# zertovitch/zip-ada

Measured on AMD Instinct MI355X. Metric: Deflate encode MB/s (Deflate_3; stream bit-exact with the CPU restatement of the reference, Ada parity unpinned), higher is better.
Workload: dtype u8

## Files before the change

### zip-ada_amd/csrc/zada_api.hip

```cpp
#include <hip/hip_runtime.h>
#include <stdint.h>
#include <stdio.h>
#include <string.h>
#include <algorithm>
#include <new>
#include <atomic>
#include <mutex>
#include <condition_variable>
#include <functional>
#include <thread>
#include "../../include/zada.h"
#include "zada_internal.h"
#include "zada_bt4.h"

struct zada_ctx { zada::Ctx c; };

namespace zada {

thread_local std::string *tls_err = nullptr;
int hip_check(Ctx *c, hipError_t e, const char *what) {
  if (e == hipSuccess) return 0;
  char buf[256];
  snprintf(buf, sizeof buf, "%s: %s", what, hipGetErrorString(e));
  if (tls_err) *tls_err = buf; else c->err = buf;
// ... 889 lines not shown
  unlzma_destroy(&z->c);
  lzma_free(&z->c);
  free_workspace(&z->c);
  for (hipEvent_t e : z->c.ev_pool) hipEventDestroy(e);
  if (z->c.stream2) hipStreamDestroy(z->c.stream2);
  if (z->c.crc_host) hipHostFree(z->c.crc_host);
  for (int b = 0; b < 2 * MAX_COPY_LANES; b++) { if (z->c.stage[b]) hipHostFree(z->c.stage[b]); if (z->c.ev_stage[b]) hipEventDestroy(z->c.ev_stage[b]); }
  for (int t = 0; t < MAX_COPY_LANES; t++) { if (z->c.stream_in[t]) hipStreamDestroy(z->c.stream_in[t]); if (z->c.ev_in[t]) hipEventDestroy(z->c.ev_in[t]); }
  if (z->c.bstage) hipHostFree(z->c.bstage);
  if (z->c.btab) hipHostFree(z->c.btab);
  if (z->c.ev_input) hipEventDestroy(z->c.ev_input);
  if (z->c.ev_out) hipEventDestroy(z->c.ev_out);
  if (z->c.ev_dlim) hipEventDestroy(z->c.ev_dlim);
  if (z->c.stream) hipStreamDestroy(z->c.stream);
  delete z;
}

zada_ctx *zada_create(int device) {
  int ndev = 0;
  if (hipGetDeviceCount(&ndev) != hipSuccess || ndev <= 0 || device < 0 || device >= ndev) return nullptr;
  if (hipSetDevice(device) != hipSuccess) return nullptr;
  zada_ctx *z = new (std::nothrow) zada_ctx();
  if (!z) return nullptr;
  z->c.device = device;
  if (hipStreamCreate(&z->c.stream) != hipSuccess ||
      hipHostMalloc((void **)&z->c.crc_host, (CRC_HOST_TOP + 64) * 4, hipHostMallocDefault) != hipSuccess ||
      hipStreamCreate(&z->c.stream2) != hipSuccess || hipEventCreateWithFlags(&z->c.ev_input, hipEventDisableTiming) != hipSuccess ||
      hipEventCreateWithFlags(&z->c.ev_out, hipEventDisableTiming) != hipSuccess || hipEventCreateWithFlags(&z->c.ev_dlim, hipEventDisableTiming) != hipSuccess) { (void)hipGetLastError(); ctx_release(z); return nullptr; }
  if (const char *e = getenv("ZADA_BUDGET")) z->c.knob_budget = atoi(e);
  if (const char *e = getenv("ZADA_INNER_BUDGET")) z->c.knob_inner_budget = atoi(e);
  if (const char *e = getenv("ZADA_LINK_RUN")) { const int v = atoi(e); if (v >= 0 && v <= 64 && !(v & (v - 1))) z->c.knob_link_run = v; }
  if (const char *e = getenv("ZADA_ATOMS_PCT")) { if (atoi(e) >= 1 && atoi(e) <= 100) z->c.knob_atoms_pct = atoi(e); }
  if (const char *e = getenv("ZADA_CD_FILTER")) z->c.knob_cd_filter = atoi(e) != 0;
  if (const char *e = getenv("ZADA_EXACT_RESPEC")) { if (atoi(e) >= 0) z->c.knob_exact_respec = atoi(e); }
  if (const char *e = getenv("ZADA_MAX_DEMAND_ROUNDS")) { if (atoi(e) > 0) z->c.knob_max_demand_rounds = atoi(e); }
  if (const char *e = getenv("ZADA_SHARD_KIB")) { if (atoi(e) >= 64 && atoi(e) % 64 == 0) z->c.knob_shard_kib = atoi(e); }
  return z;
}

void zada_destroy(zada_ctx *z) {
  if (!z) return;
  hipSetDevice(z->c.device);
  ctx_release(z);
}

const char *zada_last_error(const zada_ctx *z) { return z ? z->c.err.c_str() : "no context"; }

int zada_set_knob(zada_ctx *z, const char *name, int value) {
  if (!z || !name) return ZADA_E_INVALID;
  if (!strcmp(name, "budget")) z->c.knob_budget = value;
  else if (!strcmp(name, "inner_budget")) z->c.knob_inner_budget = value;
  else if (!strcmp(name, "link_run")) { if (value < 0 || value > 64 || (value & (value - 1))) return ZADA_E_INVALID; z->c.knob_link_run = value; }
  else if (!strcmp(name, "span_mib")) { if (value < 1 || value > 3968) return ZADA_E_INVALID; z->c.knob_span_mib = value; }
  else if (!strcmp(name, "bunzip_batch_mib")) { if (value < 16 || value > 262144) return ZADA_E_INVALID; z->c.knob_bunzip_batch_mib = value; }
  else if (!strcmp(name, "bz_batch_mib")) { if (value < 1 || value > 2048) return ZADA_E_INVALID; z->c.knob_bz_batch_mib = value; }
  else if (!strcmp(name, "bz_span_mib")) { if (value < 24 || value > 3072) return ZADA_E_INVALID; z->c.knob_bz_span_mib = value; }
  else if (!strcmp(name, "bz_batch_melems")) { if (value < 1 || value > 1536) return ZADA_E_INVALID; z->c.knob_bz_batch_melems = value; }
  else if (!strcmp(name, "bz_tail_pct")) { if (value < 0 || value > 50) return ZADA_E_INVALID; z->c.knob_bz_tail_pct = value; }
  else if (!strcmp(name, "bz_text_order")) { if (value < 0 || value > 1) return ZADA_E_INVALID; z->c.knob_bz_text_order = value; }
  else if (!strcmp(name, "bz_pipeline")) { if (value < 0 || value > 1) return ZADA_E_INVALID; z->c.knob_bz_pipeline = value; }
  else if (!strcmp(name, "bz_pipe_prio")) { if (value < 0 || value > 1) return ZADA_E_INVALID; z->c.knob_bz_pipe_prio = value; }
  else if (!strcmp(name, "bz_list_rows")) { if (value < 0 || value > 8192) return ZADA_E_INVALID; z->c.knob_bz_list_rows = value; }
  else if (!strcmp(name, "bz_split")) { if (value < 0 || value > 1) return ZADA_E_INVALID; z->c.knob_bz_split = value; }
  else if (!strcmp(name, "bz_small_wg")) { if (value < 0 || value > 1) return ZADA_E_INVALID; z->c.knob_bz_small_wg = value; }
  else if (!strcmp(name, "bz_lists")) { if (value < -1) return ZADA_E_INVALID; z->c.knob_bz_lists = value; }
  else if (!strcmp(name, "batch_mib")) { if (value < 1 || value > 1024) return ZADA_E_INVALID; z->c.knob_batch_mib = value; }
  else if (!strcmp(name, "atoms_pct")) { if (value < 1 || value > 100) return ZADA_E_INVALID; z->c.knob_atoms_pct = value; z->c.ws.cap_atoms = 0; }
  else if (!strcmp(name, "fix_stride")) { if (value < 0 || value > (int)PTOK_STRIDE) return ZADA_E_INVALID; z->c.knob_fix_stride = value; z->c.ws.cap_n = 0; }
  else if (!strcmp(name, "cd_list_cap")) { if (value < 0) return ZADA_E_INVALID; z->c.knob_cd_list_cap = value; }
  else if (!strcmp(name, "cd_filter")) { if (value < 0 || value > 1) return ZADA_E_INVALID; z->c.knob_cd_filter = value; }
  else if (!strcmp(name, "exact_respec")) { if (value < 0) return ZADA_E_INVALID; z->c.knob_exact_respec = value; }
  else if (!strcmp(name, "max_demand_rounds")) z->c.knob_max_demand_rounds = value > 0 ? value : 12;
  else if (!strcmp(name, "shard_kib")) { if (value < 64 || value % 64) return ZADA_E_INVALID; z->c.knob_shard_kib = value; }
  else if (!strcmp(name, "lzma_dict")) { if (value < 0) return ZADA_E_INVALID; z->c.knob_lzma_dict = value; }
  else if (!strcmp(name, "lzma_chunk")) { if (value < -1 || (value > 0 && value < 256)) return ZADA_E_INVALID; z->c.knob_lzma_chunk = value; }
  else if (!strcmp(name, "lzma_pool")) { if (value < 0) return ZADA_E_INVALID; z->c.knob_lzma_pool = value; }
  else if (!strcmp(name, "lzma_pool_fixed")) { if (value < 0 || value > 1) return ZADA_E_INVALID; z->c.knob_lzma_pool_fixed = value; }
  else if (!strcmp(name, "lzma_waves")) { if (value != 0 && value != 1 && value != 4) return ZADA_E_INVALID; z->c.knob_lzma_waves = value; }
  else if (!strcmp(name, "lzma_lit_mib")) { if (value < 1) return ZADA_E_INVALID; z->c.knob_lzma_lit_mib = value; }
  else if (!strcmp(name, "lzma_segment")) { if (value < -1 || (value > 0 && (value < 13 || value > 30))) return ZADA_E_INVALID; z->c.knob_lzma_segment = value; }
  else return ZADA_E_INVALID;
  return ZADA_OK;
}

constexpr int COPY_LANES = ZADA_COPY_LANES;
static_assert(COPY_LANES <= MAX_COPY_LANES, "staging buffers");
static_assert(COPY_LANES == ARR_LANES, "the arriving input's lanes use the staging buffers of copy_in's");
constexpr uint64_t COPY_MT_MIN = 64ull << 20;
static bool ensure_staging(Ctx *c, int lanes) {
  for (int b = 0; b < 2 * lanes; b++) {
    if (c->stage[b]) continue;
    if (hipHostMalloc((void **)&c->stage[b], STAGE_BYTES, hipHostMallocDefault) != hipSuccess ||
        hipEventCreateWithFlags(&c->ev_stage[b], hipEventDisableTiming) != hipSuccess) {
      if (c->stage[b]) { hipHostFree(c->stage[b]); c->stage[b] = nullptr; }
      (void)hipGetLastError();
      return false;
    }
  }
  return true;
}

static void copy_in_lane(Ctx *c, void *d_dst, const uint8_t *src, uint64_t n, int t, int T) {
  uint64_t i = 0;
// ... 1165 lines not shown
```

### zip-ada_amd/csrc/zada_internal.h

```cpp
#pragma once
#ifndef ZADA_NLEVELS
#define ZADA_NLEVELS 2
#endif
#include <hip/hip_runtime.h>
#include <stdint.h>
#include <string>
#include <functional>
#include <vector>
#include "zada_logic.h"
#include "zada_sizing.h"

namespace zada {

constexpr int ZADA_E_HIP_ = -3;

#ifndef ZADA_PCHUNK
#define ZADA_PCHUNK 512
#endif
constexpr uint32_t PCHUNK = ZADA_PCHUNK;
static_assert(PCHUNK > 258, "k_fix_forward: a 258-byte step crosses at most one chunk boundary");
constexpr uint32_t PTOK_STRIDE = PCHUNK + 640;
constexpr uint32_t FIX_STRIDE_SMALL = 128;
constexpr uint32_t CRC_CHUNK = 4096, CRC_SUB = 256;
constexpr uint64_t IN_PAD = 1024;
// ... 203 lines not shown
  void *bzd = nullptr;
  void *ulz = nullptr;
  void *lz_tab = nullptr; size_t cap_lz_tab = 0;
  void *lz_save = nullptr; size_t cap_lz_save = 0;
  void *lz_lit = nullptr; size_t cap_lz_lit = 0;
  bool lz_last_lit_hbm = false;
  int knob_lzma_lit_mib = 12288;
  int lzma_launches = 0;
  std::vector<uint8_t> lz_resume;
  bool lz_stopped = false;
  bool lz_run_stopped = false;
  uint64_t lz_last_n = 0, lz_last_out_off = 0;
  void *bt4 = nullptr;
  uint32_t bt4_buckets = 0, bt4_long = 0, bt4_overflow = 0;
  uint32_t bt4_pool_grown = 0;
  int knob_lzma_pool_fixed = 0;
  uint32_t bt4_reruns = 0;
  int knob_lzma_waves = 0;
  int knob_lzma_segment = 0;
  int knob_lzma_pool = 0;
  std::vector<hipEvent_t> ev_pool;
  std::vector<std::pair<const char *, hipEvent_t>> marks;
  std::vector<std::pair<const char *, float>> timing;
  bool timing_on = true;
  uint32_t last_nblocks = 0;
  int knob_budget = -1;
  int knob_max_demand_rounds = 12;
  int knob_atoms_pct = 50;
  int knob_fix_stride = 0;
  int knob_cd_list_cap = 0;
  int knob_cd_filter = 1;
  int knob_exact_respec = 32768;
  int knob_bz_pipe_prio = 0;
  int knob_link_run = 0;
  int knob_inner_budget = 0;
  int knob_span_mib = 2048;
  int knob_batch_mib = 512;
  int knob_bunzip_batch_mib = 8192;
  int knob_bz_batch_mib = 256;
  int knob_bz_span_mib = 1024;
  int knob_bz_text_order = 1;
  int knob_bz_tail_pct = 0;
  int knob_bz_batch_melems = 768;
  int knob_bz_lists = -1;
  int knob_bz_pipeline = 1;
  int knob_bz_list_rows = 0;
  int knob_bz_split = 1;
  int knob_bz_small_wg = 1;
  int knob_lzma_dict = 0;
  int knob_lzma_chunk = 0;
  int knob_shard_kib = 1 << 20;
  void tmark(const char *name);
  void tbegin();
  void tend();
};

extern thread_local std::string *tls_err;
int hip_check(Ctx *c, hipError_t e, const char *what);
void bz2_destroy(Ctx *c);
void crypt_destroy(Ctx *c);
void inflate_destroy(Ctx *c);
int inflate_crc_entries(Ctx *c, uint32_t E, const uint64_t *out, const uint64_t *out_len, uint32_t *regs);
void bunzip2_destroy(Ctx *c);
void unlzma_destroy(Ctx *c);
void crypt_update_keys(uint32_t keys[3], uint8_t by);
uint8_t crypt_code(const uint32_t keys[3]);
// ... 76 lines not shown
```

### zip-ada_amd/csrc/zada_lz.hip

```cpp
#include <hip/hip_runtime.h>
#include <mutex>
#include <stdint.h>
#include "zada_logic.h"
#include "zada_internal.h"
#include <chrono>
#include <stdio.h>
#include <stdlib.h>
#include <vector>

namespace zada {

typedef uint32_t __attribute__((aligned(1))) u32u;
typedef uint64_t __attribute__((aligned(1))) u64u;
#define RL(v, j) ((uint32_t)__builtin_amdgcn_readlane((int)(v), (j)))
#define RL64(v, j) ((uint64_t)RL((uint32_t)(v), (j)) | ((uint64_t)RL((uint32_t)((v) >> 32), (j)) << 32))

#ifndef ZADA_NO_XCD_MAP
__device__ __forceinline__ uint32_t xcd_block() {
  const uint32_t n = gridDim.x, full = n & ~7u, b = blockIdx.x;
  return b < full ? (b & 7u) * (full >> 3) + (b >> 3) : b;
}
#else
__device__ __forceinline__ uint32_t xcd_block() { return blockIdx.x; }
#endif
// ... 92 lines not shown
    for (int k = 0; k < w; k++) base += wsum[k];
    uint32_t run = base + incl - s;
    for (int k = 0; k < PER; k++) { const int idx = tid * PER + k; cnt[(idx & 15) * NDIG + (idx >> 4)] = run; run += v[k]; }
  }
  lds_barrier();
  SP_STAMP(2);
#pragma unroll
  for (int it = 0; it < 32; it++) {
    if (it * 64 < rem) {
      const uint32_t wd = word(it), d = (wd >> (16 + SHIFT)) & (uint32_t)(NDIG - 1);
      dst[mycnt[d] + ((rk[it >> 1] >> (16 * (it & 1))) & 0xFFFFu)] = wd;
    }
  }
  lds_barrier();
  SP_STAMP(3);
}

constexpr uint32_t DIST3_CONTINUE = 0xFFFF, DIST3_HEADCHK = 0xFFFE, DIST3_CONT_FIRST = 0xFFFD, DISTL_CONTINUE = 0x8000;
#ifndef ZADA_WALK_CAP
#define ZADA_WALK_CAP 16
#endif
constexpr uint32_t DISTL_GAVEUP = 0x7FFF, WALK_CAP = ZADA_WALK_CAP;
static_assert(MAX_DIST < 0x7FFF, "the give-up marker is no distance");
constexpr uint32_t HEAVY_STRIDE = 2048, HEAVY_CAP = HEAVY_STRIDE - 1;
static_assert(MAX_DIST < 0x8000, "continue markers of the planes");
constexpr int PL_LDS = 144 * 1024 + 64, PL_LDS_RUNS = 160 * 1024, PL_PREV_OFF = 131072;
constexpr int PL_HB_OFF = PL_PREV_OFF + 12288;
static_assert(PL_PREV_OFF + 32768 <= PL_LDS_RUNS, "k_prev_links: LDS map of the fused cross links");
template <bool RUNS>
__global__ void __launch_bounds__(1024) k_prev_links(const uint8_t *__restrict__ in, Layout L, int kfull, int kquarter,
                                                     LevelPtrs lv,
                                                     uint16_t *__restrict__ S3, uint8_t *__restrict__ T3, uint32_t *__restrict__ bsc3,
                                                     DistPlanes dp, RunPtrs rp, unsigned long long *__restrict__ dbg, uint32_t *__restrict__ segmax,
                                                     uint16_t *__restrict__ heavy, uint32_t seg0, uint32_t run_len, uint32_t seg_end) {
#ifdef ZADA_PL_STATS
  unsigned long long tprev = clock64(); int tph = 8;
#define PL_STAMP() do { lds_barrier(); if (threadIdx.x == 0) { unsigned long long t = clock64(); atomicAdd(&dbg[tph], t - tprev); tprev = t; } tph++; } while (0)
#else
#define PL_STAMP() do {} while (0)
#endif
  extern __shared__ __attribute__((aligned(16))) uint8_t smem[];
  uint16_t *A = (uint16_t *)smem;
  uint16_t *B = A + 32768;
  uint32_t *AB = (uint32_t *)smem;
  uint32_t *cnt = (uint32_t *)(B + 32768);
  uint32_t *wsum = cnt + 4096;
  const int tid = threadIdx.x, lane = tid & 63, w = tid >> 6;
  const uint8_t *pbL = smem + PL_PREV_OFF;
#pragma unroll 1
  for (uint32_t jrun = 0; jrun < (RUNS ? run_len : 1u); jrun++) {
  const uint64_t seg = (uint64_t)blockIdx.x * run_len + jrun + seg0, base = seg * 32768ull;
  if (seg >= seg_end) break;
  const uint32_t m = lay_inserted(L, seg);
  const bool first_seg = lay_first(L, seg);
  const bool fused = RUNS && jrun > 0 && !first_seg;
  const bool prev_first = fused && lay_first(L, seg - 1);

#ifdef ZADA_PL_STATS
  tph = 8;
#endif
  uint32_t *bsc = bsc3 + seg * 32768ull;
  uint16_t *s3 = S3 + seg * 32768ull;
  uint8_t *t3 = T3 + seg * 32768ull;
  uint16_t *hvy = heavy + seg * HEAVY_STRIDE;
  const uint32_t heavy_thr = kquarter / 2 > 0 ? (uint32_t)kquarter / 2 : 1u;
#ifdef ZADA_OLD_INIT
  for (int l = 0; l < NLEVELS; l++) {
    uint16_t *tail = lv.tails[l] + seg * 65536ull;
    for (int i = tid; i < 65536 / 8; i += 1024) ((uint4 *)tail)[i] = make_uint4(~0u, ~0u, ~0u, ~0u);
  }
  for (uint32_t e = tid; e < m; e += 1024) dp.dlim[base + e] = 0xFFFFFFFFu;
#endif
  const uint8_t *sin = in + base;
  PL_STAMP();
  uint32_t *F = cnt;
  uint16_t *LW = (uint16_t *)(cnt + 1040);
  const uint8_t *sb = (const uint8_t *)A;
  uint16_t *P = B;
  auto lb8 = [&](uint32_t e) -> uint64_t {
    const uint32_t *wp = (const uint32_t *)(sb + (e & ~3u));
    const uint32_t a = wp[0], b = wp[1], s = e & 3u;
    return (uint64_t)__builtin_amdgcn_alignbyte(b, a, s) | ((uint64_t)(b >> (8u * s)) << 32);
  };
  static_assert(3 + NLEVELS <= 5 + 1, "lb8 yields five valid bytes");
#pragma unroll 1
  for (int lvl = 0; lvl <= NLEVELS; lvl++) {
    const int L = 3 + lvl;
    uint32_t i0 = (uint32_t)w * 2048 + lane;
    asm volatile("" : "+v"(i0));
    const int rem = (int)m - (int)i0;

    {
      {
        uint32_t key[16];
#pragma unroll
        for (int k = 0; k < 16; k++) key[k] = 0;
        const uint32_t sh = i0 & 3u;
        auto build = [&](auto wp) {
#pragma unroll
          for (int g8 = 0; g8 < 4; g8++) {
            uint32_t wa[8], wb[8], wc[8];
#pragma unroll
            for (int q = 0; q < 8; q++) { const int it = g8 * 8 + q; wa[q] = wp[it * 16]; wb[q] = wp[it * 16 + 1]; wc[q] = wp[it * 16 + 2]; }
#pragma unroll
            for (int q = 0; q < 8; q++) {
              const int it = g8 * 8 + q;
              const uint64_t v = (uint64_t)__builtin_amdgcn_alignbyte(wb[q], wa[q], sh) | ((uint64_t)__builtin_amdgcn_alignbyte(wc[q], wb[q], sh) << 32);
              uint32_t k = (lvl == 0) ? hash3_of(v) : hashL_of(v, L);
              if (!(it * 64 < rem)) k = 0;
              key[it >> 1] |= k << (16 * (it & 1));
            }
          }
        };
        if (lvl == 0) {
          build((const uint32_t *)(sin + (i0 & ~3u)));
          for (int i = tid; i < 32768 / 4; i += 1024) ((uint4 *)bsc)[i] = make_uint4(0, 0, 0, 0);
          if (RUNS) {
            for (int l = 0; l < NLEVELS; l++) {
              uint16_t *tl = lv.tails[l] + seg * 65536ull;
              for (int i = tid; i < 65536 / 8; i += 1024) ((uint4 *)tl)[i] = make_uint4(~0u, ~0u, ~0u, ~0u);
            }
          }
        } else build((const uint32_t *)(sb + (i0 & ~3u)));
        sort_pass<256, 0, true>(key, AB, cnt, wsum, i0, rem);
      }
      uint32_t pr[32];
      {
        const uint32_t *pp = AB + i0;
#pragma unroll
        for (int it = 0; it < 32; it++) pr[it] = (it * 64 < rem) ? pp[it * 64] : 0u;
      }
      if (lvl == 0) sort_pass<128, 8, false>(pr, AB, cnt, wsum, i0, rem);
      else sort_pass<256, 8, false>(pr, AB, cnt, wsum, i0, rem);
    }
    if (lvl == 0) __syncthreads();
    PL_STAMP();
    uint16_t *tail = lvl > 0 ? lv.tails[lvl - 1] + seg * 65536ull : nullptr;
    const bool want_runs = lvl == 0 || lvl == NLEVELS;
    uint32_t ed[32];
    const bool keyed = RUNS && fused && lvl > 0;
    uint32_t *HB = (uint32_t *)(smem + PL_HB_OFF);
    uint32_t firstmask = 0;
    if (keyed) HB[tid] = 0;
    {
      const uint32_t *pp = AB + i0;
      uint32_t *pf = F + (i0 >> 5);
#pragma unroll
      for (int it = 0; it < 32; it++) {
        uint32_t x = 0;
        bool first = false;
        if (it * 64 < rem) {
          const uint32_t p0 = pp[it * 64], e = p0 & 0xFFFFu, k = p0 >> 16;
          uint32_t pm = 0;
          first = i0 + it * 64 == 0;
          if (!first) { pm = pp[it * 64 - 1]; first = (pm >> 16) != k; }
          const bool last = (it * 64 + 1 == rem) || ((pp[it * 64 + 1] >> 16) != k);
          uint32_t d = 0;
          if (!first) { const uint32_t e0 = pm & 0xFFFFu; if (!(first_seg && e0 == 0)) d = e - e0; }
          else if (keyed) d = k;
          firstmask |= (uint32_t)first << it;
          x = e | ((uint32_t)last << 15) | (d << 16);
          if (lvl > 0 && last) tail[k] = (uint16_t)e;
        }
        ed[it] = x;
        if (want_runs) {
          const unsigned long long mk = __ballot(first);
          if (lane == 0) { pf[it * 2] = (uint32_t)mk; pf[it * 2 + 1] = (uint32_t)(mk >> 32); }
        }
// ... 107 lines not shown
              P[eb[q]] = (t != 0xFFFFu && dx <= (uint32_t)MAX_DIST && !(prev_first && t == 0)) ? (uint16_t)dx : (uint16_t)0;
            }
          }
        }
        lds_barrier();
        if (lvl < NLEVELS) { for (uint32_t i = tid; i < (m + 16 + 15) / 16; i += 1024) ((uint4 *)A)[i] = ((const uint4 *)sin)[i]; }
      }
      uint16_t *prevl = lv.prev[lvl - 1];
      for (uint32_t i = tid; i < (m + 7) / 8; i += 1024) ((uint4 *)(prevl + base))[i] = ((const uint4 *)P)[i];
    }
    PL_STAMP();
    if (lvl < NLEVELS) {
      const uint64_t lmask = (1ull << (8 * L)) - 1ull;
      uint16_t *plane = dp.d[lvl] + base;
      auto dflt_of = [&](uint32_t e, uint32_t q) -> uint32_t {
        if (first_seg) return 0u;
        if (lvl == 0) return e < (uint32_t)TOO_FAR ? (q == e ? DIST3_CONT_FIRST : DIST3_CONTINUE) : (q == e ? DIST3_HEADCHK : 0u);
        if (RUNS && fused) {
          const uint32_t step = P[q];
          if (step == 0) return 0u;
          const uint32_t t = q + 32768u - step, d = e + 32768u - t;
          if (d > (uint32_t)MAX_DIST) return 0u;
          if (t <= 32768u - 4u) {
            const uint32_t theirs = lds_u32_tail(pbL, t);
            if (theirs == (uint32_t)lb8(e)) return d;
          }
        }
        return DISTL_CONTINUE | (e - q);
      };
      static_assert(NLEVELS <= 2, "the candidate compare of the fused cross links takes four bytes");
      constexpr uint32_t QCAP = 4000;
      uint32_t *Qa = (uint32_t *)(smem + 32800), *Qb = Qa + QCAP;
      uint32_t *qn = RUNS ? (uint32_t *)(smem + 32800 + 8 * QCAP) : wsum;
      static_assert(32800 + 8 * QCAP + 8 <= 65536, "queues and their counters behind the staged bytes");
      const unsigned long long ltm = (1ull << lane) - 1ull;
      if (tid < 2) qn[tid] = 0;
      if (RUNS && fused && lvl > 0) {
        const uint4 *bs = (const uint4 *)(in + base - 32768ull);
        for (int i = tid; i < 32768 / 16; i += 1024) ((uint4 *)(smem + PL_PREV_OFF))[i] = bs[i];
      }
      lds_barrier();
      auto walk = [&](uint32_t e, uint32_t &q, uint64_t mine, uint32_t maxs, uint32_t &dl) -> bool {
        uint32_t step = P[q];
        for (uint32_t sidx = 0; sidx < maxs; sidx++) {
          if (step - 1u >= q) { dl = dflt_of(e, q); return true; }
          q -= step;
          const uint32_t dist = e - q;
          step = P[q];
          const uint64_t theirs = lb8(q);
          if (dist > (uint32_t)(lvl == 0 ? TOO_FAR : MAX_DIST)) { dl = 0; return true; }
          if ((theirs & lmask) == mine) { dl = dist; return true; }
        }
        return false;
      };
      auto push = [&](bool pend, uint32_t entry, uint32_t *dstq, uint32_t *cntp) -> bool {
        const unsigned long long mk = __ballot(pend);
        if (mk == 0) return true;
        uint32_t b0 = 0;
        const int leader = __ffsll((long long)mk) - 1;
        if (lane == leader) b0 = atomicAdd(cntp, (uint32_t)__popcll(mk));
        b0 = __shfl(b0, leader);
        const uint32_t idx = b0 + __popcll(mk & ltm);
        if (pend && idx < QCAP) { dstq[idx] = entry; return true; }
        return !pend;
      };
      const bool capped = lvl > 0 && !first_seg && WALK_CAP > 0;
      const uint32_t maxs_last = capped ? WALK_CAP : 1u << 30;
      for (uint32_t e0 = 0; e0 < m; e0 += 4096) {
        uint32_t ee[4], st[4];
        uint64_t mn[4], th[4];
        bool ex[4];
#pragma unroll
        for (int j = 0; j < 4; j++) { const uint32_t e = e0 + 1024u * j + tid; ex[j] = e < m; ee[j] = ex[j] ? e : 0u; }
#pragma unroll
        for (int j = 0; j < 4; j++) { mn[j] = lb8(ee[j]) & lmask; st[j] = P[ee[j]]; }
#pragma unroll
        for (int j = 0; j < 4; j++) th[j] = lb8(st[j] <= ee[j] ? ee[j] - st[j] : ee[j]) & lmask;
        uint32_t pw[4] = {0, 0, 0, 0};
        if (RUNS && fused && lvl > 0) {
#pragma unroll
          for (int j = 0; j < 4; j++) {
            const uint32_t t = st[j] > ee[j] ? ee[j] + 32768u - st[j] : 0u, tr = t <= 32768u - 4u ? t : 0u;
            pw[j] = lds_u32_tail(pbL, tr);
          }
        }
#pragma unroll
        for (int j = 0; j < 4; j++) {
          const uint32_t e = ee[j], step = st[j];
          uint32_t dl = 0, q = e;
          bool pend = false;
          if (!(ex[j] && step - 1u < e)) {
            if (RUNS && fused && lvl > 0) {
              if (step != 0) dl = (e + 32768u - step <= 32768u - 4u && pw[j] == (uint32_t)mn[j]) ? step : DISTL_CONTINUE;
            } else dl = dflt_of(e, e);
          }
          if (ex[j] && step - 1u < e) {
            q = e - step;
            if (lvl == 0) {
              if (th[j] == mn[j] && (step <= (uint32_t)TOO_FAR || step == (uint32_t)MAX_DIST)) dl = step;
              else if (step >= (uint32_t)TOO_FAR) dl = 0;
              else pend = true;
            } else {
              if (step > (uint32_t)MAX_DIST) dl = 0;
              else if (th[j] == mn[j]) dl = step;
              else pend = true;
            }
          }
          if (!push(pend, e | (q << 16), Qa, &qn[0])) { if (!walk(e, q, mn[j], maxs_last, dl)) dl = DISTL_GAVEUP; pend = false; }
          if (ex[j] && !pend) plane[e] = (uint16_t)dl;
        }
      }
      lds_barrier();
      PL_STAMP();
      for (int cur = 0;; cur ^= 1) {
        const uint32_t nq = qn[cur] < QCAP ? qn[cur] : QCAP;
        if (nq == 0) break;
#ifdef ZADA_PL_STATS
        if (tid == 0 && lvl == 1) { atomicAdd(&dbg[24], 1ull); atomicAdd(&dbg[25], (unsigned long long)nq); if (nq <= 1024) atomicAdd(&dbg[26], (unsigned long long)nq); if (cur == 0 && qn[0] > QCAP) atomicAdd(&dbg[30], (unsigned long long)(qn[0] - QCAP)); }
        unsigned long long tq0 = clock64();
#endif
        lds_barrier();
        if (tid == 0) qn[cur ^ 1] = 0;
        lds_barrier();
        if (nq > 1024) {
          static_assert(QCAP <= 4096, "four entries per lane cover the queue");
          const uint32_t *Qs = cur ? Qb : Qa;
          uint32_t e4[4], q4[4], st4[4], dl4[4];
          uint64_t mn4[4];
          bool val[4], act[4];
#pragma unroll
          for (int j = 0; j < 4; j++) {
            const uint32_t idx = 1024u * j + tid;
            val[j] = idx < nq;
            const uint32_t ent = Qs[val[j] ? idx : 0u];
            e4[j] = ent & 0x7FFFu; q4[j] = ent >> 16; act[j] = val[j]; dl4[j] = 0;
          }
#pragma unroll
          for (int j = 0; j < 4; j++) { mn4[j] = lb8(e4[j]) & lmask; st4[j] = P[q4[j]]; }
          for (int sidx = 0; sidx < 8; sidx++) {
            uint32_t qx[4], ns[4];
            uint64_t th[4];
#pragma unroll
            for (int j = 0; j < 4; j++) {
// ... 304 lines not shown
    const uint64_t lo = p - (uint64_t)MAX_DIST > first ? p - (uint64_t)MAX_DIST : first;
    const uint32_t mine = *(const u32u *)(in + p);
    uint32_t found = 0;
    for (uint64_t hi = p; hi > lo && !found; hi = hi - lo > 2048 ? hi - 2048 : lo) {
      uint64_t v[8];
#pragma unroll
      for (int u = 0; u < 8; u++) {
        const uint64_t q0 = hi - 256ull * (uint64_t)(u + 1) + 4ull * lane;
        v[u] = (q0 < hi && q0 + 3 >= lo) ? *(const u64u *)(in + q0) : 0ull;
      }
#pragma unroll
      for (int u = 0; u < 8; u++) {
        const uint64_t q0 = hi - 256ull * (uint64_t)(u + 1) + 4ull * lane;
        uint32_t mk = 0;
        if (q0 < hi && q0 + 3 >= lo) {
#pragma unroll
          for (int j = 0; j < 4; j++) if ((uint32_t)(v[u] >> (8 * j)) == mine && q0 + (uint64_t)j >= lo && q0 + (uint64_t)j < hi) mk |= 1u << j;
        }
        const unsigned long long m = __ballot(mk != 0);
        if (m && !found) {
          const int top = 63 - __builtin_clzll(m);
          const uint32_t tm = RL(mk, top);
          const uint64_t q = hi - 256ull * (uint64_t)(u + 1) + 4ull * (uint64_t)top + (uint64_t)(31 - __builtin_clz(tm));
          found = (uint32_t)(p - q);
        }
      }
    }
    if (lane == 0) dp.d[1][p] = (uint16_t)found;
  }
}

__global__ void __launch_bounds__(256) k_bucket_limits(Layout L, int kfull, int kquarter, const uint16_t *__restrict__ S3,
                                                       const uint32_t *__restrict__ bsc3, uint32_t *__restrict__ dlim, uint32_t *__restrict__ dlim_bits, const uint32_t *__restrict__ segmax,
                                                       const uint16_t *__restrict__ heavy, uint32_t seg0) {
  __shared__ uint32_t list[2048];
  __shared__ uint32_t nlist;
  __shared__ uint32_t lbits[1024];
  const uint64_t seg = (uint64_t)blockIdx.x + seg0, base = seg * 32768ull;
  const int tid = threadIdx.x;
  const bool has_prev = !lay_first(L, seg);
  {
    const uint32_t mo = segmax[seg], mp = has_prev ? segmax[seg - 1] : 0u;
    if (mo == 0 || mo - 1 + mp < (uint32_t)kquarter) return;
  }
  for (int i = tid; i < 1024; i += 256) lbits[i] = 0;
  auto flush_bits = [&]() { __syncthreads(); for (int i = tid; i < 1024; i += 256) { const uint32_t w = lbits[i]; if (w) dlim_bits[(base >> 5) + i] = w; } };
  const uint32_t *own = bsc3 + base, *prv = has_prev ? bsc3 + base - 32768 : nullptr;
  const uint16_t *s3 = S3 + base, *p3 = has_prev ? S3 + base - 32768 : nullptr;
  auto qualifies = [&](uint32_t h) -> bool {
    const uint32_t c = own[h] >> 16, cp = prv ? prv[h] >> 16 : 0u;
    return c > 0 && c - 1 + cp >= (uint32_t)kquarter;
  };
  auto process = [&]() {
    const uint32_t nl = nlist < 2048 ? nlist : 2048;
    for (uint32_t li = 0; li < nl; li++) {
      const uint32_t h = list[li];
      const uint32_t st = own[h] & 0xFFFF, c = own[h] >> 16;
      const uint32_t pst = prv ? prv[h] & 0xFFFF : 0u, cp = prv ? prv[h] >> 16 : 0u;
      const uint32_t r0 = (uint32_t)kquarter > cp ? (uint32_t)kquarter - cp : 0u;
      for (uint32_t r = r0 + tid; r < c; r += 256) {
        const uint32_t e = s3[st + r];
        uint32_t lim[2];
        const uint32_t ks[2] = {(uint32_t)kfull, (uint32_t)kquarter};
        for (int t = 0; t < 2; t++) {
          const uint32_t k = ks[t];
          uint64_t d = 0xFFFF;
          if (r >= k) d = e - s3[st + r - k];
          else if (cp >= k - r) d = (base + e) - (base - 32768 + p3[pst + cp - (k - r)]);
          lim[t] = d < 0xFFFF ? (uint32_t)d : 0xFFFFu;
        }
        dlim[base + e] = lim[0] | (lim[1] << 16);
        atomicOr(&lbits[e >> 5], 1u << (e & 31u));
      }
    }
  };
  const uint32_t heavy_thr = kquarter / 2 > 0 ? (uint32_t)kquarter / 2 : 1u;
  const uint16_t *ho = heavy + seg * HEAVY_STRIDE, *hp = has_prev ? heavy + (seg - 1) * HEAVY_STRIDE : nullptr;
  const uint32_t no = ho[0], np = hp ? hp[0] : 0u;
  if (no != 0xFFFFu && np != 0xFFFFu) {
    for (int phase = 0; phase < 2; phase++) {
      if (tid == 0) nlist = 0;
      __syncthreads();
      const uint16_t *hl = phase == 0 ? ho : hp;
      const uint32_t nh = phase == 0 ? no : np;
      for (uint32_t i = tid; i < nh; i += 256) {
        const uint32_t h = hl[1 + i];
        if (phase == 1 && (own[h] >> 16) >= heavy_thr) continue;
        if (qualifies(h)) { const uint32_t k = atomicAdd(&nlist, 1u); if (k < 2048) list[k] = h; }
      }
      __syncthreads();
      process();
      __syncthreads();
    }
    flush_bits();
    return;
  }
  for (uint32_t h0 = 0; h0 < 32768; h0 += 2048) {
    if (tid == 0) nlist = 0;
    __syncthreads();
    for (uint32_t h = h0 + tid; h < h0 + 2048; h += 256) {
      if (qualifies(h)) { const uint32_t k = atomicAdd(&nlist, 1u); if (k < 2048) list[k] = h; }
    }
    __syncthreads();
    process();
    __syncthreads();
// ... 1000 lines not shown
      if (int rg = job.grow_atoms(cnt, &dst_atoms, &dst_apos)) return rg;
    }
    if (cnt) hipLaunchKernelGGL(k_literal_atoms, dim3(2048), dim3(256), 0, st, W.in + job.tok_lo, cnt, dst_atoms, dst_apos, job.apos_bias + job.tok_lo);
    res->ntok = (uint32_t)cnt;
    res->exit = ExitState{(uint32_t)hi, SYNC_F};
    return hip_check(c, hipGetLastError(), "k_literal_atoms");
  }
  const LzConfig cfg = lz_config(level);
  const Layout L{job.segend, n};
  const uint64_t n_ins = job.segend ? n : (n >= 2 ? n - 2 : 0);
  const uint32_t nseg = (uint32_t)((n_ins + 32767) / 32768);
  c->tmark("lz:begin");
  if (!c->lz_attrs_set) {
    hipFuncSetAttribute((const void *)k_prev_links<true>, hipFuncAttributeMaxDynamicSharedMemorySize, PL_LDS_RUNS);
    hipFuncSetAttribute((const void *)k_prev_links<false>, hipFuncAttributeMaxDynamicSharedMemorySize, PL_LDS);
    hipFuncSetAttribute((const void *)k_cross_links, hipFuncAttributeMaxDynamicSharedMemorySize, CL_LDS_PLANE);
    hipFuncSetAttribute((const void *)k_match, hipFuncAttributeMaxDynamicSharedMemorySize, MATCH_LDS);
    hipFuncSetAttribute((const void *)k_match_demand, hipFuncAttributeMaxDynamicSharedMemorySize, DM_LDS);
    c->lz_attrs_set = true;
  }
  LevelPtrs lv;
  DistPlanes dpl;
  RunPtrs rpt; rpt.S = W.SK; rpt.idx = W.idxK; rpt.cnt = W.cntK;
  for (int l = 0; l < NLEVELS; l++) dpl.d[l] = W.dplane[l];
  dpl.dlim = W.dlim; dpl.dlim_bits = W.dlim_bits;
  if (nseg > 0) {
    for (int l = 0; l < NLEVELS; l++) { lv.prev[l] = W.lprev[l]; lv.tails[l] = W.ltails[l]; }
#ifndef ZADA_OLD_INIT
    hipEventRecord(c->ev_dlim, st);
    hipStreamWaitEvent(c->stream2, c->ev_dlim, 0);
    hipMemsetAsync(W.dlim_bits, 0, (size_t)(n / 32 + 2) * 4, c->stream2);
    hipEventRecord(c->ev_dlim, c->stream2);
#endif
    uint32_t R = 1;
    if (c->knob_link_run > 0) R = (uint32_t)c->knob_link_run;
    else {
      while (R < 16 && nseg / (2 * R) >= 1024) R *= 2;
      if (job.need && R > 8) R = 8;
    }
    if ((R & (R - 1)) || R > 64) { c->err = "link_run is not a power of two up to 64"; return -1; }
    auto prev_links = [&](uint32_t s0, uint32_t s1) {
      if (R > 1) hipLaunchKernelGGL(k_prev_links<true>, dim3((s1 - s0 + R - 1) / R), dim3(1024), PL_LDS_RUNS, st, W.in, L, cfg.chain, cfg.chain >> 2, lv,
                                    W.S3, W.T3, W.bsc3, dpl, rpt, (unsigned long long *)W.dbg, W.segmax, W.heavy, s0, R, s1);
      else hipLaunchKernelGGL(k_prev_links<false>, dim3(s1 - s0), dim3(1024), PL_LDS, st, W.in, L, cfg.chain, cfg.chain >> 2, lv,
                              W.S3, W.T3, W.bsc3, dpl, rpt, (unsigned long long *)W.dbg, W.segmax, W.heavy, s0, 1u, s1);
    };
    auto cross_links = [&](uint32_t from, uint32_t to) {
      const uint32_t first = (from + R - 1) / R * R;
      if (first < to) hipLaunchKernelGGL(k_cross_links, dim3((to - first + R - 1) / R, NLEVELS), dim3(1024), CL_LDS_PLANE, st, W.in, L, lv, dpl, first, R);
    };
    static_assert(BLOOM_WORDS == 4096, "Workspace::bloom4 is sized in zada_api.hip");
    auto cross_dist = [&]() {
      const uint32_t nb = (uint32_t)((n_ins - 32768 + CD_THREADS - 1) / CD_THREADS);
      if (!c->knob_cd_filter) {
        hipLaunchKernelGGL(k_cross_dist<CD_ALL>, dim3(nb), dim3(CD_THREADS), 0, st, W.in, L, lv, W.S3, W.T3, W.bsc3, dpl, (uint64_t)32768, (uint64_t)n, CdTail{nullptr, nullptr, W.n_changed + 4, 0u, nullptr, W.n_changed + 5, 0u});
        return;
      }
      hipMemsetAsync(W.n_changed + 4, 0, 4, st);
      hipLaunchKernelGGL(k_bloom4, dim3(nseg - 1), dim3(256), 0, st, W.in, L, W.bloom4, 0u);
      hipMemsetAsync(W.n_changed + 5, 0, 4, st);
      const uint32_t lcap = c->knob_cd_list_cap > 0 && (uint64_t)c->knob_cd_list_cap < W.cd_cap ? (uint32_t)c->knob_cd_list_cap : (uint32_t)W.cd_cap;
      const CdTail tl{W.bloom4, W.cd_list, W.n_changed + 4, lcap, W.cd_list + W.cd_cap, W.n_changed + 5, lcap / 4};
      hipLaunchKernelGGL(k_cross_dist<CD_SWEEP>, dim3(nb), dim3(CD_THREADS), 0, st, W.in, L, lv, W.S3, W.T3, W.bsc3, dpl, (uint64_t)32768, (uint64_t)n, tl);
      hipLaunchKernelGGL(k_cross_dist<CD_LIST>, dim3((uint32_t)((W.cd_cap + CD_THREADS - 1) / CD_THREADS)), dim3(CD_THREADS), 0, st, W.in, L, lv, W.S3, W.T3, W.bsc3, dpl, (uint64_t)0, (uint64_t)n, tl);
      hipLaunchKernelGGL(k_cross_scan, dim3(2048), dim3(256), 0, st, W.in, L, dpl, tl);
    };
    if (job.need) {
      constexpr uint32_t PIECE = 2048;
      static_assert(PIECE % 64 == 0, "pieces start at multiples of every run length (a power of two up to 64)");
      constexpr double SLOW_PIECE_S = 2.0e-3;
      uint32_t cl_from = 1;
      auto cross_links_upto = [&](uint32_t s1) {
        if (s1 > cl_from) cross_links(cl_from, s1);
        if (s1 > cl_from) cl_from = s1;
      };
      auto t_prev = std::chrono::steady_clock::now();
      for (uint32_t s0 = 0; s0 < nseg;) {
        const uint32_t s1 = s0 + PIECE < nseg ? s0 + PIECE : nseg;
        const uint64_t upto = (uint64_t)s1 * 32768 + 64 < n ? (uint64_t)s1 * 32768 + 64 : n;
        if (int rn = job.need(upto)) return rn;
        const auto t_now = std::chrono::steady_clock::now();
        const bool slow = s0 > 0 && std::chrono::duration<double>(t_now - t_prev).count() >= SLOW_PIECE_S;
        t_prev = t_now;
        prev_links(s0, s1);
#ifndef ZADA_OLD_INIT
        if (s0 == 0) hipStreamWaitEvent(st, c->ev_dlim, 0);
#endif
        if (slow) cross_links_upto(s1);
        hipLaunchKernelGGL(k_bucket_limits, dim3(s1 - s0), dim3(256), 0, st, L, cfg.chain, cfg.chain >> 2, W.S3, W.bsc3, W.dlim, W.dlim_bits, W.segmax, W.heavy, s0);
        s0 = s1;
      }
      if (int rn = job.need(n)) return rn;
      cross_links_upto(nseg);
      if (nseg > 1) cross_dist();
    } else
    prev_links(0, nseg);
#ifndef ZADA_OLD_INIT
    if (!job.need) hipStreamWaitEvent(st, c->ev_dlim, 0);
#endif
#ifdef ZADA_PL_STATS
    { unsigned long long h[32]; hipMemcpy(h, W.dbg, sizeof h, hipMemcpyDeviceToHost); fprintf(stderr, "[prev_links cycles/segment] init %.0f |", (double)h[8] / nseg); for (int q = 9; q < 9 + 4 * (NLEVELS + 1) - 1; q++) fprintf(stderr, " %.0f", (double)h[q] / nseg); fprintf(stderr, "  (per level 3..: sort, links, first candidates, queue rounds)\n"); fprintf(stderr, "[level 4 walks per segment] rounds %.2f  entries %.1f  entries of the last round %.1f  hops there %.1f (max %llu over all segments; walks over 64 hops %.3f)  first-queue overflow %.1f  cycles of the last round %.0f\n", (double)h[24] / nseg, (double)h[25] / nseg, (double)h[26] / nseg, (double)h[27] / nseg, h[28], (double)h[29] / nseg, (double)h[30] / nseg, (double)h[31] / nseg); hipMemset(W.dbg, 0, 256);
      unsigned long long sd[8]; hipMemcpyFromSymbol(sd, HIP_SYMBOL(g_sort_dbg), sizeof sd); fprintf(stderr, "[sort_pass cycles/segment, all six passes] clear %.0f  rank (LDS atomics) %.0f  scan %.0f  scatter %.0f\n", (double)sd[0] / nseg, (double)sd[1] / nseg, (double)sd[2] / nseg, (double)sd[3] / nseg); for (int q = 0; q < 8; q++) sd[q] = 0; hipMemcpyToSymbol(HIP_SYMBOL(g_sort_dbg), sd, sizeof sd); }
#endif
    c->tmark("prev_links");
    if (!job.need) {
      if (nseg > 1) {
        cross_links(1, nseg);
        cross_dist();
      }
      hipLaunchKernelGGL(k_bucket_limits, dim3(nseg), dim3(256), 0, st, L, cfg.chain, cfg.chain >> 2, W.S3, W.bsc3, W.dlim, W.dlim_bits, W.segmax, W.heavy, 0u);
    }
  }
#ifdef ZADA_CD_STATS
  { unsigned long long h[16]; hipDeviceSynchronize(); hipMemcpyFromSymbol(h, HIP_SYMBOL(g_cd_dbg), sizeof h);
    fprintf(stderr, "[k_cross_dist level-4 walks] %llu walks (%.1f %% of the positions), %llu steps (%.2f per walk), found %llu (%.1f %%), no step %llu, > 8 steps %llu, > 64 steps %llu, steps of the walks that found nothing %llu, gave-up restarts %llu\n",
            h[0], 100.0 * h[0] / n, h[1], (double)h[1] / (h[0] ? h[0] : 1), h[2], 100.0 * h[2] / (h[0] ? h[0] : 1), h[3], h[4], h[5], h[6], h[7]);
    fprintf(stderr, "[k_cross_dist level-4 walks] > 32 steps %llu, > 128 %llu, > 256 %llu, > 512 %llu, > 1024 %llu, longest %llu\n", h[8], h[9], h[10], h[11], h[12], h[13]);
    for (int q = 0; q < 16; q++) h[q] = 0; hipMemcpyToSymbol(HIP_SYMBOL(g_cd_dbg), h, sizeof h); }
#endif
  c->tmark("cross_links");
  const uint32_t nbm = (uint32_t)((n + MB - 1) / MB);
  const uint32_t nch = (uint32_t)((n + PCHUNK - 1) / PCHUNK);
  const int max_rounds = c->knob_max_demand_rounds;
  int budget_env = c->knob_budget >= 0 ? c->knob_budget : (n < (2u << 20) ? 0 : n < (512u << 20) ? 8 : 6);
  if (budget_env < 1) budget_env = 1 << 20;
  const uint32_t nbd = (uint32_t)((n + DMB - 1) / DMB);
  hipMemsetAsync(W.blk_demand, 0, (size_t)nbd * 4, st);
  hipMemsetAsync(W.dbits, 0, (size_t)nbd * (DMB / 8), st);
  hipMemsetAsync(W.n_demand, 0, 4, st);
  hipLaunchKernelGGL(k_match, dim3(nbm), dim3(1024), MATCH_LDS, st, W.in, L, W.lprev[NLEVELS - 1], dpl, W.M, cfg.nice,
                     budget_env, (unsigned long long *)W.dbg, W.lprev[0], budget_env > c->knob_inner_budget ? c->knob_inner_budget : 0);
  c->tmark("match");
  ParseIO io; io.in = W.in; io.n = n; io.M = W.M; io.cfg = cfg; io.segend = job.segend;
  DemandMarker dm; dm.M = W.M; dm.blk_demand = W.blk_demand; dm.n_demand = W.n_demand; dm.by = M_BYSPEC; dm.dbits = W.dbits;
  DemandMarker dmf = dm; dmf.by = 0;
  int rounds = 0, demand_rounds = 0;
  bool valve_used = false;
  static const bool round_stats = getenv("ZADA_ROUND_STATS") != nullptr;
  const ExitState entry0 = job.entry_known ? job.entry : ExitState{0, SYNC_F};
  const uint32_t kE = job.entry_known ? (entry0.pos / PCHUNK < nch ? entry0.pos / PCHUNK : nch) : 0u;
  hipMemsetAsync(W.n_changed + 6, 0, 4, st);
  bool restart = false, first_again = false;
  for (bool first = true;; first = false) {
// ... 109 lines not shown
```

Baseline: 9427.

## Derive level-3 distances lazily from level-4 results and fix heavy buckets later

Reorders the per-segment level processing so level 4 runs before level 3. Positions whose level-4 distance is already valid reuse it as their level-3 distance, and only the unsettled positions are compacted into an LDS list and walked at level 3. k_bucket_limits then re-scans the capped heavy buckets and corrects the level-3 distance wherever a nearer 3-byte match exists, which keeps the output bit-exact. This saves level-3 chain walks at the cost of an extra compaction pass, more LDS queue space, and extra input reads in the bucket-limits kernel.

```diff
diff --git a/zip-ada_amd/csrc/zada_api.hip b/zip-ada_amd/csrc/zada_api.hip
--- a/zip-ada_amd/csrc/zada_api.hip
+++ b/zip-ada_amd/csrc/zada_api.hip
@@ -945,6 +945,7 @@
   if (const char *e = getenv("ZADA_LINK_RUN")) { const int v = atoi(e); if (v >= 0 && v <= 64 && !(v & (v - 1))) z->c.knob_link_run = v; }
   if (const char *e = getenv("ZADA_ATOMS_PCT")) { if (atoi(e) >= 1 && atoi(e) <= 100) z->c.knob_atoms_pct = atoi(e); }
   if (const char *e = getenv("ZADA_CD_FILTER")) z->c.knob_cd_filter = atoi(e) != 0;
+  if (const char *e = getenv("ZADA_D3_LAZY")) z->c.knob_d3_lazy = atoi(e) != 0;
   if (const char *e = getenv("ZADA_EXACT_RESPEC")) { if (atoi(e) >= 0) z->c.knob_exact_respec = atoi(e); }
   if (const char *e = getenv("ZADA_MAX_DEMAND_ROUNDS")) { if (atoi(e) > 0) z->c.knob_max_demand_rounds = atoi(e); }
   if (const char *e = getenv("ZADA_SHARD_KIB")) { if (atoi(e) >= 64 && atoi(e) % 64 == 0) z->c.knob_shard_kib = atoi(e); }
@@ -982,6 +983,7 @@
   else if (!strcmp(name, "fix_stride")) { if (value < 0 || value > (int)PTOK_STRIDE) return ZADA_E_INVALID; z->c.knob_fix_stride = value; z->c.ws.cap_n = 0; }
   else if (!strcmp(name, "cd_list_cap")) { if (value < 0) return ZADA_E_INVALID; z->c.knob_cd_list_cap = value; }
   else if (!strcmp(name, "cd_filter")) { if (value < 0 || value > 1) return ZADA_E_INVALID; z->c.knob_cd_filter = value; }
+  else if (!strcmp(name, "d3_lazy")) { if (value < 0 || value > 1) return ZADA_E_INVALID; z->c.knob_d3_lazy = value; }
   else if (!strcmp(name, "exact_respec")) { if (value < 0) return ZADA_E_INVALID; z->c.knob_exact_respec = value; }
   else if (!strcmp(name, "max_demand_rounds")) z->c.knob_max_demand_rounds = value > 0 ? value : 12;
   else if (!strcmp(name, "shard_kib")) { if (value < 64 || value % 64) return ZADA_E_INVALID; z->c.knob_shard_kib = value; }
diff --git a/zip-ada_amd/csrc/zada_internal.h b/zip-ada_amd/csrc/zada_internal.h
--- a/zip-ada_amd/csrc/zada_internal.h
+++ b/zip-ada_amd/csrc/zada_internal.h
@@ -259,6 +259,7 @@
   int knob_cd_filter = 1;
   int knob_exact_respec = 32768;
   int knob_bz_pipe_prio = 0;
+  int knob_d3_lazy = 1;
   int knob_link_run = 0;
   int knob_inner_budget = 0;
   int knob_span_mib = 2048;
diff --git a/zip-ada_amd/csrc/zada_lz.hip b/zip-ada_amd/csrc/zada_lz.hip
--- a/zip-ada_amd/csrc/zada_lz.hip
+++ b/zip-ada_amd/csrc/zada_lz.hip
@@ -148,7 +148,7 @@
                                                      LevelPtrs lv,
                                                      uint16_t *__restrict__ S3, uint8_t *__restrict__ T3, uint32_t *__restrict__ bsc3,
                                                      DistPlanes dp, RunPtrs rp, unsigned long long *__restrict__ dbg, uint32_t *__restrict__ segmax,
-                                                     uint16_t *__restrict__ heavy, uint32_t seg0, uint32_t run_len, uint32_t seg_end) {
+                                                     uint16_t *__restrict__ heavy, uint32_t seg0, uint32_t run_len, uint32_t seg_end, uint32_t lazy3) {
 #ifdef ZADA_PL_STATS
   unsigned long long tprev = clock64(); int tph = 8;
 #define PL_STAMP() do { lds_barrier(); if (threadIdx.x == 0) { unsigned long long t = clock64(); atomicAdd(&dbg[tph], t - tprev); tprev = t; } tph++; } while (0)
@@ -168,6 +168,7 @@
   const uint64_t seg = (uint64_t)blockIdx.x * run_len + jrun + seg0, base = seg * 32768ull;
   if (seg >= seg_end) break;
   const uint32_t m = lay_inserted(L, seg);
+  const uint32_t m4 = lay_end(L, seg) - base - 2 > 32768ull ? 32768u : (m > 0 ? m - 1u : 0u);
   const bool first_seg = lay_first(L, seg);
   const bool fused = RUNS && jrun > 0 && !first_seg;
   const bool prev_first = fused && lay_first(L, seg - 1);
@@ -199,9 +200,14 @@
     return (uint64_t)__builtin_amdgcn_alignbyte(b, a, s) | ((uint64_t)(b >> (8u * s)) << 32);
   };
   static_assert(3 + NLEVELS <= 5 + 1, "lb8 yields five valid bytes");
+  static_assert(NLEVELS == 2, "order of the levels with d3_lazy");
 #pragma unroll 1
-  for (int lvl = 0; lvl <= NLEVELS; lvl++) {
+  for (int li = 0; li <= NLEVELS; li++) {
+    const int lvl = lazy3 && li < 2 ? 1 - li : li;
     const int L = 3 + lvl;
+#ifdef ZADA_PL_STATS
+    tph = 9 + 4 * lvl;
+#endif
     uint32_t i0 = (uint32_t)w * 2048 + lane;
     asm volatile("" : "+v"(i0));
     const int rem = (int)m - (int)i0;
@@ -228,7 +234,7 @@
             }
           }
         };
-        if (lvl == 0) {
+        if (li == 0) {
           build((const uint32_t *)(sin + (i0 & ~3u)));
           for (int i = tid; i < 32768 / 4; i += 1024) ((uint4 *)bsc)[i] = make_uint4(0, 0, 0, 0);
           if (RUNS) {
@@ -249,7 +255,7 @@
       if (lvl == 0) sort_pass<128, 8, false>(pr, AB, cnt, wsum, i0, rem);
       else sort_pass<256, 8, false>(pr, AB, cnt, wsum, i0, rem);
     }
-    if (lvl == 0) __syncthreads();
+    if (li == 0) __syncthreads();
     PL_STAMP();
     uint16_t *tail = lvl > 0 ? lv.tails[lvl - 1] + seg * 65536ull : nullptr;
     const bool want_runs = lvl == 0 || lvl == NLEVELS;
@@ -423,7 +429,7 @@
       constexpr uint32_t QCAP = 4000;
       uint32_t *Qa = (uint32_t *)(smem + 32800), *Qb = Qa + QCAP;
       uint32_t *qn = RUNS ? (uint32_t *)(smem + 32800 + 8 * QCAP) : wsum;
-      static_assert(32800 + 8 * QCAP + 8 <= 65536, "queues and their counters behind the staged bytes");
+      static_assert(32800 + 8 * QCAP + 16 <= 65536, "queues and their counters behind the staged bytes");
       const unsigned long long ltm = (1ull << lane) - 1ull;
       if (tid < 2) qn[tid] = 0;
       if (RUNS && fused && lvl > 0) {
@@ -457,12 +463,42 @@
       };
       const bool capped = lvl > 0 && !first_seg && WALK_CAP > 0;
       const uint32_t maxs_last = capped ? WALK_CAP : 1u << 30;
-      for (uint32_t e0 = 0; e0 < m; e0 += 4096) {
+      const bool lazyl = lvl == 0 && lazy3 != 0;
+      uint16_t *UL = (uint16_t *)cnt;
+#pragma unroll 1
+      for (uint32_t c0 = 0; c0 < m; c0 += lazyl ? 8192u : 32768u) {
+      uint32_t nu = m;
+      if (lazyl) {
+        uint32_t *un = &qn[2 + ((c0 >> 13) & 1u)];
+        const uint16_t *pl4 = dp.d[1] + base;
+        if (tid == 0) *un = 0;
+        lds_barrier();
+        uint32_t d4[8];
+#pragma unroll
+        for (int j = 0; j < 8; j++) { const uint32_t e = c0 + 1024u * j + tid; d4[j] = e < m ? (uint32_t)pl4[e] : 0u; }
+#pragma unroll
+        for (int j = 0; j < 8; j++) {
+          const uint32_t e = c0 + 1024u * j + tid;
+          const bool settled = d4[j] - 1u < (uint32_t)MAX_DIST - 1u && e < m4;
+          if (settled) plane[e] = (uint16_t)d4[j];
+          const unsigned long long mk = __ballot(e < m && !settled);
+          if (mk) {
+            uint32_t b0 = 0;
+            const int leader = __ffsll((long long)mk) - 1;
+            if (lane == leader) b0 = atomicAdd(un, (uint32_t)__popcll(mk));
+            b0 = __shfl(b0, leader);
+            if (e < m && !settled) UL[b0 + __popcll(mk & ltm)] = (uint16_t)e;
+          }
+        }
+        lds_barrier();
+        nu = *un;
+      }
+      for (uint32_t e0 = 0; e0 < nu; e0 += 4096) {
         uint32_t ee[4], st[4];
         uint64_t mn[4], th[4];
         bool ex[4];
 #pragma unroll
-        for (int j = 0; j < 4; j++) { const uint32_t e = e0 + 1024u * j + tid; ex[j] = e < m; ee[j] = ex[j] ? e : 0u; }
+        for (int j = 0; j < 4; j++) { const uint32_t e = e0 + 1024u * j + tid; ex[j] = e < nu; ee[j] = ex[j] ? (lazyl ? (uint32_t)UL[e] : e) : 0u; }
 #pragma unroll
         for (int j = 0; j < 4; j++) { mn[j] = lb8(ee[j]) & lmask; st[j] = P[ee[j]]; }
 #pragma unroll
@@ -500,6 +536,7 @@
           if (!push(pend, e | (q << 16), Qa, &qn[0])) { if (!walk(e, q, mn[j], maxs_last, dl)) dl = DISTL_GAVEUP; pend = false; }
           if (ex[j] && !pend) plane[e] = (uint16_t)dl;
         }
+      }
       }
       lds_barrier();
       PL_STAMP();
@@ -870,13 +907,14 @@
 
 __global__ void __launch_bounds__(256) k_bucket_limits(Layout L, int kfull, int kquarter, const uint16_t *__restrict__ S3,
                                                        const uint32_t *__restrict__ bsc3, uint32_t *__restrict__ dlim, uint32_t *__restrict__ dlim_bits, const uint32_t *__restrict__ segmax,
-                                                       const uint16_t *__restrict__ heavy, uint32_t seg0) {
+                                                       const uint16_t *__restrict__ heavy, uint32_t seg0, const uint8_t *__restrict__ in, uint16_t *__restrict__ d3p,
+                                                       const uint16_t *__restrict__ d4p) {
   __shared__ uint32_t list[2048];
   __shared__ uint32_t nlist;
   __shared__ uint32_t lbits[1024];
   const uint64_t seg = (uint64_t)blockIdx.x + seg0, base = seg * 32768ull;
   const int tid = threadIdx.x;
-  const bool has_prev = !lay_first(L, seg);
+  const bool has_prev = !lay_first(L, seg), prev_first = has_prev && lay_first(L, seg - 1);
   {
     const uint32_t mo = segmax[seg], mp = has_prev ? segmax[seg - 1] : 0u;
     if (mo == 0 || mo - 1 + mp < (uint32_t)kquarter) return;
@@ -909,6 +947,25 @@
         }
         dlim[base + e] = lim[0] | (lim[1] << 16);
         atomicOr(&lbits[e >> 5], 1u << (e & 31u));
+        if (in) {
+          const uint32_t v3 = d3p[base + e];
+          if (v3 == (uint32_t)d4p[base + e] && v3 - 1u < (uint32_t)MAX_DIST - 1u) {
+            const uint32_t my24 = *(const u32u *)(in + base + e) & 0xFFFFFFu;
+            uint32_t d3 = 0;
+            bool open = true;
+            for (uint32_t j = r; j > 0 && open;) {
+              const uint32_t q = s3[st + --j], d = e - q;
+              if (d > (uint32_t)TOO_FAR || (!has_prev && q == 0)) open = false;
+              else if ((*(const u32u *)(in + base + q) & 0xFFFFFFu) == my24) { d3 = d; open = false; }
+            }
+            for (uint32_t j = cp; j > 0 && open;) {
+              const uint32_t q = p3[pst + --j], d = e + 32768u - q;
+              if (d > (uint32_t)TOO_FAR || (prev_first && q == 0)) open = false;
+              else if ((*(const u32u *)(in + base - 32768 + q) & 0xFFFFFFu) == my24) { d3 = d; open = false; }
+            }
+            if (d3 != v3) d3p[base + e] = (uint16_t)d3;
+          }
+        }
       }
     }
   };
@@ -1975,6 +2032,7 @@
     hipMemsetAsync(W.dlim_bits, 0, (size_t)(n / 32 + 2) * 4, c->stream2);
     hipEventRecord(c->ev_dlim, c->stream2);
 #endif
+    const uint32_t lazy3 = c->knob_d3_lazy && (uint32_t)((cfg.chain >> 2) / 2) * HEAVY_CAP >= 32768u ? 1u : 0u;
     uint32_t R = 1;
     if (c->knob_link_run > 0) R = (uint32_t)c->knob_link_run;
     else {
@@ -1984,9 +2042,9 @@
     if ((R & (R - 1)) || R > 64) { c->err = "link_run is not a power of two up to 64"; return -1; }
     auto prev_links = [&](uint32_t s0, uint32_t s1) {
       if (R > 1) hipLaunchKernelGGL(k_prev_links<true>, dim3((s1 - s0 + R - 1) / R), dim3(1024), PL_LDS_RUNS, st, W.in, L, cfg.chain, cfg.chain >> 2, lv,
-                                    W.S3, W.T3, W.bsc3, dpl, rpt, (unsigned long long *)W.dbg, W.segmax, W.heavy, s0, R, s1);
+                                    W.S3, W.T3, W.bsc3, dpl, rpt, (unsigned long long *)W.dbg, W.segmax, W.heavy, s0, R, s1, lazy3);
       else hipLaunchKernelGGL(k_prev_links<false>, dim3(s1 - s0), dim3(1024), PL_LDS, st, W.in, L, cfg.chain, cfg.chain >> 2, lv,
-                              W.S3, W.T3, W.bsc3, dpl, rpt, (unsigned long long *)W.dbg, W.segmax, W.heavy, s0, 1u, s1);
+                              W.S3, W.T3, W.bsc3, dpl, rpt, (unsigned long long *)W.dbg, W.segmax, W.heavy, s0, 1u, s1, lazy3);
     };
     auto cross_links = [&](uint32_t from, uint32_t to) {
       const uint32_t first = (from + R - 1) / R * R;
@@ -2030,7 +2088,7 @@
         if (s0 == 0) hipStreamWaitEvent(st, c->ev_dlim, 0);
 #endif
         if (slow) cross_links_upto(s1);
-        hipLaunchKernelGGL(k_bucket_limits, dim3(s1 - s0), dim3(256), 0, st, L, cfg.chain, cfg.chain >> 2, W.S3, W.bsc3, W.dlim, W.dlim_bits, W.segmax, W.heavy, s0);
+        hipLaunchKernelGGL(k_bucket_limits, dim3(s1 - s0), dim3(256), 0, st, L, cfg.chain, cfg.chain >> 2, W.S3, W.bsc3, W.dlim, W.dlim_bits, W.segmax, W.heavy, s0, lazy3 ? W.in : nullptr, W.dplane[0], W.dplane[1]);
         s0 = s1;
       }
       if (int rn = job.need(n)) return rn;
@@ -2051,7 +2109,7 @@
         cross_links(1, nseg);
         cross_dist();
       }
-      hipLaunchKernelGGL(k_bucket_limits, dim3(nseg), dim3(256), 0, st, L, cfg.chain, cfg.chain >> 2, W.S3, W.bsc3, W.dlim, W.dlim_bits, W.segmax, W.heavy, 0u);
+      hipLaunchKernelGGL(k_bucket_limits, dim3(nseg), dim3(256), 0, st, L, cfg.chain, cfg.chain >> 2, W.S3, W.bsc3, W.dlim, W.dlim_bits, W.segmax, W.heavy, 0u, lazy3 ? W.in : nullptr, W.dplane[0], W.dplane[1]);
     }
   }
 #ifdef ZADA_CD_STATS
```

Measured after the change: 9295. -1.4%, worse.
